# aosprey/mckpp-f90

Measured on AMD Instinct MI355X. Metric: column-steps/s at 1e5 cols x 60 levels, 1/2/4/8 GPU; % HBM roofline, higher is better.
Workload: dtype f64

## Files before the change

### mckpp_f90_amd/csrc/mckpp_device.h

```cpp
#pragma once
#include <hip/hip_runtime.h>
#include <stdint.h>

#define MCKPP_CS 24
#define MCKPP_CI 8
#define MCKPP_XS 8
enum { XS_RELAX_SST = 0, XS_SST0, XS_FCORR_TWOD, XS_RELAX_SAL, XS_RELAX_OCNT };

enum {
  CS_F = 0, CS_SSURF, CS_SREF, CS_SSREF, CS_OCDEPTH,
  CS_SFLUX1, CS_SFLUX2, CS_SFLUX3, CS_SFLUX4, CS_SFLUX5, CS_SFLUX6,
  CS_HMIXD0, CS_HMIXD1, CS_HMIX, CS_KMIX, CS_UREF, CS_VREF, CS_TREF,
  CS_RESET, CS_DAMPU, CS_DAMPV, CS_FREEZE, CS_FCORR, CS_SPARE1
};
enum { CI_OLD = 0, CI_NEW, CI_JERLOV, CI_INITFLAG, CI_STATUS, CI_NPASS, CI_LOCEAN, CI_IPT };

enum { MCKPP_MODE_STEP = 0, MCKPP_MODE_INIT = 1, MCKPP_MODE_PASS = 2, MCKPP_MODE_VMIX = 3 };

template <class T> using mckpp_ptr_plain = T *;
template <class T> using mckpp_ptr_global = __attribute__((address_space(1))) T *;

template <template <class> class P>
struct mckpp_kparams_t {
  int nz, nzp1, ncol, ld;
  int ntime, itermax, mode, diag;
  int L_SSref, LDD, clim_present;
  int l2pre;
  double hmixtolfrac, dto, grav, vonk, sice;
  double Vtc;
  double cg;
  double dm_nz;
  P<const double> zm, hm, tri0, tri1;
  P<const double> swfrac_tab;
  P<const double> swdk_tab;
  int ldc;
  int LRI;
  int solver_mode;
  int l3cap;
  P<const double> wtab;
  P<double> U, V, T, S;
  P<double> Us[2], Vs[2], Ts[2], Ss[2];
  P<const double> U_init, V_init;
  P<double> cs;
  P<int> ci;
  P<int> qhead;
  int nsteps_launch;
  int nqueues;
  int xcc_queue[16];
  P<const double> series;
  int series_rec0, ndtocn, l_rest;
  double flsn, el;
  P<int> qowner;
  P<int> done;
  P<unsigned long long> dbg;
  int ext, L_RELAX_SST, L_RELAX_CALCONLY, L_FCORR, L_FCORR_WITHZ, L_SFCORR, L_SFCORR_WITHZ;
  int L_RELAX_SAL, L_RELAX_OCNT, L_NO_FREEZE, L_NO_ISOTHERM, L_DAMP_CURR, iso_bot, dt_uvdamp, maxmodeadv;
  double iso_thresh;
  P<const double> dm;
  P<const double> hsum;
  P<const double> xs;
  P<const double> fcorr_withz, sfcorr_withz, ocnT_clim, sal_clim;
  P<double> tinc_fcorr, sinc_fcorr, ocnTcorr, scorr;
  P<const int> adv_i;
  P<const double> adv_d;
  P<double> rho, cp, buoy, talpha, sbeta, difm, difs, dift, ghat;
  P<double> wU1, wU2, wX1, wX2, wX3, wXNT1, Rig, dbloc, Shsq;
  P<double> scratch;
  size_t scratch_doubles;
  P<int> sync;
  int solo_after;
  int view_kmax;
  int solo_limit;
};
using mckpp_kparams = mckpp_kparams_t<mckpp_ptr_plain>;
using mckpp_kparams_dev = mckpp_kparams_t<mckpp_ptr_global>;
static_assert(sizeof(mckpp_kparams) == sizeof(mckpp_kparams_dev), "same layout");

struct mckpp_launch_info { int nblocks, threads, max_blocks_per_cu; size_t lds_bytes; };

hipError_t mckpp_launch_column_kernel_ps(const mckpp_kparams &p, const mckpp_kparams *dp, int num_cu,
                                         hipStream_t stream, mckpp_launch_info *info);
size_t mckpp_ps_scratch_doubles(int nzp1, int variant, int num_cu);
hipError_t mckpp_launch_xcc_probe(unsigned *mask, hipStream_t stream);
hipError_t mckpp_launch_eos_batch(int64_t n, const double *s, const double *t, const double *p,
                                  double *alpha, double *beta, double *sig0, double *cp,
                                  hipStream_t stream);
hipError_t mckpp_launch_div_batch(int64_t n, const double *num, const double *den, double *q, hipStream_t stream);
hipError_t mckpp_launch_exp_batch(int64_t n, const double *x, double *y, hipStream_t stream);
hipError_t mckpp_launch_bottomtemp(const mckpp_kparams &p, const double *bt, hipStream_t stream);
hipError_t mckpp_launch_fluxes(const mckpp_kparams &p, int ntime, const double *f8, int l_rest, double flsn,
                               double el, hipStream_t stream);
struct mckpp_pack_list { int nd, ni; int dslot[MCKPP_CS]; int islot[MCKPP_CI]; };
hipError_t mckpp_launch_unpack_sflux(const double *slabs, const int *ipt, double *cs, int64_t ncol, int64_t npts, hipStream_t stream);
hipError_t mckpp_launch_pack_records(const double *cs, const int *ci, const int *ipt, int64_t ncol, int64_t npts,
                                     const mckpp_pack_list &l, double *dout, int *iout, hipStream_t stream);
hipError_t mckpp_launch_out_sample(const double *src, int src_ld, int src_off, const double *cs, int add_sref,
                                   int64_t ncol, int nlev, int ld_out, double *sum, double *mn, double *mx, int first,
                                   double *inst, hipStream_t stream);
hipError_t mckpp_launch_window_mean(const double *sum, double *out, size_t n, double count, hipStream_t stream);
hipError_t mckpp_launch_gather_rows(const double *src3d, int64_t npts, int nlev, int lev_off,
                                    const int *ipt, int64_t ncol, double *dst, int ld, int dst_off,
                                    hipStream_t stream);
hipError_t mckpp_launch_scatter_rows(const double *src, int ld, int src_off, const int *ipt,
                                     int64_t ncol, double *dst3d, int64_t npts, int nlev, int lev_off,
                                     hipStream_t stream);
```

### mckpp_f90_amd/csrc/mckpp_kernels_ps.hip

```cpp
#include "mckpp_colmath.h"

#include <cstdio>
#include <cstdlib>
#include <type_traits>

namespace {

using namespace mckpp_dev;

enum { PS_EMPTY = 0, PS_ACTIVE = 1, PS_DONE = 2, PS_WAIT = 3  };
enum { F_NONE = 0, F_TRAP = 1, F_FINAL = 2 };

enum {
  C_B0 = 0, C_B0SOL, C_USTAR, C_UFRAC, C_UCUBE, C_HEK, C_WU01, C_WU02, C_WX01, C_WX02, C_WXNT0, C_UREFNZ, C_VREFNZ,
  C_RHO0CP0, C_RRC, X_T1 , X_S1, X_RHOH2O, X_RHOB,
  C_F, C_HMIXE, C_HMIXN, C_HBL, C_RHBL, C_STABLE, C_BFSFC, C_CASEA,
  C_GAT1, C_DAT1 = C_GAT1 + 3, C_DKM1 = C_DAT1 + 3,
  C_SREF = C_DKM1 + 3, C_SSURF, C_OCDEPTH, C_SFLUX1, C_SFLUX2, C_SFLUX3, C_SFLUX4, C_SFLUX5, C_SFLUX6,
  C_T1X ,
  C_JRFAC = C_T1X + 2, C_JA1, C_JA2, C_JRA1, C_JRA2 ,
  C_COUNT_USED,
  C_COUNT = C_COUNT_USED | 1
};
enum {
// ... 893 lines not shown
    c_t1[i] = p.tri1[i];
    c_rdz[i] = rcp_refine(p.zm[i] - p.zm[i + 1]);
    c_dtohk[i] = p.dto / p.hm[i];
  }
  if (tid == 0) { c_misc[0] = rcp_refine(p.hm[1]); c_misc[1] = rcp_refine(p.vonk); }
  for (int i = tid; i < W0 * I_COUNT; i += blockDim.x) sirec0[i] = 0;
  if (tid < 32) s_flags[tid] = tid == 3 ? nz : 0;
  const int mgr = 0;
  const int my_xcc = __builtin_amdgcn_s_getreg(((4 - 1) << 11) | 20 ) & 15;
  if (tid == 0 && p.nsteps_launch > 1) {
    int q = p.xcc_queue[my_xcc];
    if (q >= 0) {
      const int prev = atomicCAS((int *)p.qowner + q, 0, my_xcc + 1);
      if (prev != 0 && prev != my_xcc + 1) q = -1;
    }
    s_flags[7] = q;
  }

  const int nthreads = blockDim.x;
  const int nitems = W0 * L;
  const int nhelp = nthreads > 64 ? nthreads - 64 : 64, tid2 = nthreads > 64 ? tid - 64 : tid;
  const int nitems_lm = W0 * nzp1;
  const unsigned Wmagic = W0 > 1 ? 0xFFFFFFFFu / (unsigned)W0 + 1u : 0u;
  const int kmax_view = nthreads > 64 ? min(min((nthreads - 64) / L, (int)S_MAPMAX), p.view_kmax > 0 ? p.view_kmax : (int)S_MAPMAX) : 0;
  const bool solo_ok = kmax_view >= 1;
  const bool solo_perm = W0 == 1 && solo_ok;
  const bool solo_dyn = p.mode == MCKPP_MODE_STEP && solo_ok && !solo_perm && p.solo_limit > 0;
  bool sparse = false;
  int it0 = tid, it0_lm = tid, trip_base = nthreads;
  auto set_view = [&](int kv) {
    sparse = kv > 0;
    if (!sparse) { it0 = tid; it0_lm = tid; trip_base = nthreads; return; }
    trip_base = 0x20000000;
    const int i0 = tid - 64;
    it0 = 0x3fffffff; it0_lm = 0x3fffffff;
    if (i0 >= 0 && i0 < kv * L) {
      const int vs = (int)__umulhi((unsigned)i0, Lmagic);
      it0 = s_flags[S_MAP + vs] * L + (i0 - vs * L);
    }
    if (i0 >= 0 && i0 < kv * nzp1) {
      const int lk = i0 / kv;
      it0_lm = lk * W0 + s_flags[S_MAP + (i0 - lk * kv)];
    }
  };
  if (solo_perm && tid == 0) { s_flags[S_KVIEW] = 1; s_flags[S_MAP] = 0; }
  __syncthreads();
  if (solo_perm) set_view(1);

  const double lambda = 0.5;
  const double epsln16 = 1.e-16, Ricr = 0.30, eps01 = 0.1, cekman = 0.7, cmonob = 1.0, epsln20 = 1.e-20;
  const bool do_ocnint = p.mode == MCKPP_MODE_STEP || p.mode == MCKPP_MODE_PASS;
  const bool flux_diag = p.mode == MCKPP_MODE_STEP || p.mode == MCKPP_MODE_INIT;
  double rU = 0.0, rV = 0.0, rT = 0.0, rS = 0.0, r2U = 0.0, r2V = 0.0, r2T = 0.0, r2S = 0.0;
  const int LS = ps_scratch_ld(nzp1);
  const auto scr0 = p.scratch + (size_t)blockIdx.x * (size_t)W0 * (size_t)(4 * LS);

#define PS_ITEMS_PRAGMA _Pragma("clang loop unroll(disable)")
#define FOR_ITEMS                                                                         \
  PS_ITEMS_PRAGMA                                                                         \
  for (int it_ = it0, t_ = 0; it_ < nitems; it_ = tid2 >= 0 ? trip_base + t_ * nhelp + tid2 : nitems, ++t_) { \
    const int slot = (int)__umulhi((unsigned)it_, Lmagic);                                \
    const int k = it_ - slot * L + 1;                                                     \
    int *const si = sirec + slot * I_COUNT;                                               \
    if (!si[I_ACT]) continue;                                                             \
    double *const my = slots + slot * SS;                                                 \
    double *const sc = screc + slot * C_COUNT;                                            \
    const int col = si[I_COL];                                                            \
    const bool act = k <= nzp1, actz = k <= nz, virt1 = k == nzp1 + 1, virt2 = k == nzp1 + 2; \
    const bool is1 = k == 1, isnz = k == nz, isnzp1 = k == nzp1;                          \
    const int kr = act ? k : 1;                                                           \
    const size_t ro = (size_t)col * p.ld;                                                 \
    const auto xs_ = scr0 + (size_t)slot * (size_t)(4 * LS) + (kr - 1);    \
    const int first_ = t_;         \
    auto row = [&](int a) -> strided<ROWS> { return strided<ROWS>{my + a}; };             \
    (void)sc; (void)actz; (void)virt1; (void)virt2; (void)is1; (void)isnz; (void)isnzp1; (void)kr; (void)ro; (void)xs_; (void)first_; (void)row;
#define END_ITEMS }
#define FOR_ITEMS_BY_LEVEL                                                                \
  for (int j_ = it0_lm, t_ = 0; j_ < nitems_lm; j_ = tid2 >= 0 ? trip_base + t_ * nhelp + tid2 : nitems_lm, ++t_) { \
    const int it_ = t_ == 0 ? j_ : nitems_lm - 1 - (j_ - nthreads);                       \
    const int k = (W == 1 ? it_ : (int)__umulhi((unsigned)it_, Wmagic)) + 1;    \
    const int slot = it_ - (k - 1) * W;                                                   \
    int *const si = sirec + slot * I_COUNT;                                               \
    if (!si[I_ACT]) continue;                                                             \
    double *const my = slots + slot * SS;                                                 \
    double *const sc = screc + slot * C_COUNT;                                            \
    const int col = si[I_COL];                                                            \
    const bool act = true, actz = k <= nz;                                                \
    const bool is1 = k == 1, isnz = k == nz, isnzp1 = k == nzp1;                          \
    const size_t ro = (size_t)col * p.ld;                                                 \
    auto row = [&](int a) -> strided<ROWS> { return strided<ROWS>{my + a}; };             \
    (void)sc; (void)act; (void)actz; (void)is1; (void)isnz; (void)isnzp1; (void)ro; (void)row;

#define FOR_ITEMS_RISING                                                                  \
  for (int it_ = it0_lm, t_ = 0; it_ < nitems_lm; it_ = tid2 >= 0 ? trip_base + t_ * nhelp + tid2 : nitems_lm, ++t_) { \
    const int k = (W == 1 ? it_ : (int)__umulhi((unsigned)it_, Wmagic)) + 1;              \
    const int slot = it_ - (k - 1) * W;                                                   \
    int *const si = sirec + slot * I_COUNT;                                               \
    if (!si[I_ACT]) continue;                                                             \
    double *const my = slots + slot * SS;                                                 \
    double *const sc = screc + slot * C_COUNT;                                            \
    const bool actz = k <= nz, is1 = k == 1, isnz = k == nz;                              \
    auto row = [&](int a) -> strided<ROWS> { return strided<ROWS>{my + a}; };             \
    (void)sc; (void)actz; (void)is1; (void)isnz; (void)row;

  auto M0 = [&]() {
    int lane = lane_k; asm volatile("" : "+v"(lane));
// ... 323 lines not shown
              if (npass_try < p.itermax) { msc[C_HMIXE] = hmixn; go_on = true; }
              else if (hmixn > hmixe) { msc[C_HMIXE] = hmixn; go_on = true; }
            }
            if (!go_on) {
              if (npass_try > (p.itermax + 1)) status |= 2;
              fin = F_TRAP;
              msi[I_NVIOL] = 0;
            }
          }
          msi[I_MAYBE_NEXT] = (npass_try >= 3 && (iconv >= 2 || npass_try + 1 >= p.itermax)) ? 1 : 0;
        }
        msi[I_STATUS] = status; msi[I_NPASS_TRY] = npass_try; msi[I_ICONV] = iconv;
        msi[I_FIN] = fin;
        msi[I_L1A] = (l1_ahead && fin == F_NONE) ? 1 : 0;
        f_any = fin != F_NONE;
      }
    }
    const unsigned long long m = __ballot(f_any);
    if (lane == 0) s_flags[1] = m != 0ull ? 1 : 0;
#ifdef MCKPP_PS_STAMPS
    {
      const bool sg = lane < W && sirec[lane * I_COUNT + I_STATE] == PS_ACTIVE && sirec[lane * I_COUNT + I_ACT] && sirec[lane * I_COUNT + I_STRAG];
      const int n = __popcll(__ballot(sg));
      const int nact = __popcll(__ballot(lane < W && sirec[lane * I_COUNT + I_STATE] == PS_ACTIVE && sirec[lane * I_COUNT + I_ACT]));
      if (lane == 0 && n > 0) { atomicAdd((int *)p.sync + (sparse ? 1 : 2), n); atomicAdd((int *)p.sync + (sparse ? 3 : 4), 1); atomicAdd((int *)p.sync + (sparse ? 5 : 6), nact); }
    }
#endif
    if (solo_dyn && !sparse) {
      const int f_kv = s_flags[S_KVIEW], f_drain = s_flags[S_DRAIN];
      if (f_kv == 0 && f_drain) {
        const int *msi = sirec + (lane < W ? lane : 0) * I_COUNT;
        const bool on = lane < W && msi[I_STATE] == PS_ACTIVE && msi[I_ACT];
        const bool ok = on && msi[I_FIN] == F_NONE && (msi[I_STRAG] || msi[I_NPASS_TRY] > p.solo_after);
        const unsigned long long m_on = __ballot(on), m_ok = __ballot(ok);
        const int kn = __popcll(m_on);
        if (kn >= 1 && kn <= kmax_view && m_ok == m_on) {
          if (on) s_flags[S_MAP + __popcll(m_on & ((1ull << lane) - 1ull))] = lane;
          if (lane == 0) s_flags[S_GOVIEW] = kn;
        }
      }
    }
  };
  auto G_late = [&]() {
    int lane = lane_k; asm volatile("" : "+v"(lane));
    if (lane < W) {
      int *msi = sirec + lane * I_COUNT;
      if (msi[I_ACT]) {
        if (p.mode != MCKPP_MODE_INIT && msi[I_BAD]) msi[I_STATUS] = msi[I_STATUS] | 1;
        msi[I_BAD] = 0;
        msi[I_TINY] = 0;
        msi[I_MAYBE] = msi[I_MAYBE_NEXT];
      }
    }
  };

  auto ext_rhs = [&](double *my, const int *si, int col, int k, int kmixe, double To_k, double So_k, double &rhsT,
                     double &rhsS) {
    const double dto = p.dto;
    const auto xs = p.xs + (size_t)col * MCKPP_XS;
    const double rhok = my[k * ROWS + Q_RHO], cpk = my[k * ROWS + Q_CP];
    const size_t oin = (size_t)col * p.ld + (k - 1);
    if (k == 1) {
      if (p.L_RELAX_SST && !p.L_FCORR_WITHZ && !p.L_FCORR) {
        const double relax_sst = xs[XS_RELAX_SST], SST0 = xs[XS_SST0];
        double fc = 0.0;
        if (relax_sst > 1.e-10) {
          if (!p.L_RELAX_CALCONLY) rhsT = rhsT + dto * relax_sst * (SST0 - To_k) * p.dm[kmixe] / c_hm[1];
          fc = relax_sst * (SST0 - To_k) * p.dm[kmixe] * rhok * cpk;
        }
        p.cs[(size_t)col * MCKPP_CS + CS_FCORR] = fc;
      }
      if (p.L_FCORR && !p.L_RELAX_SST && !p.L_FCORR_WITHZ)
        rhsT = rhsT + dto * xs[XS_FCORR_TWOD] / (rhok * cpk * c_hm[1]);
    }
    double tinc = 0.;
    if (p.L_FCORR_WITHZ && !p.L_FCORR) tinc = dto * p.fcorr_withz[oin] / (rhok * cpk);
    if (p.L_RELAX_OCNT) tinc = tinc + dto * xs[XS_RELAX_OCNT] * (p.ocnT_clim[oin] - To_k);
    rhsT = rhsT + tinc;
    const double ocnTcorr = tinc * rhok * cpk / dto;
    const auto ai = p.adv_i + (size_t)col * (p.maxmodeadv + 1);
    const auto ad = p.adv_d + (size_t)col * (p.maxmodeadv + 1);
    const int nmode = ai[0];
    const int nzi = nz, km = kmixe;
    for (int im = 0; im < nmode; ++im) {
      const int mode = ai[1 + im];
      if (mode <= 0) continue;
      const double fact = dto * ad[im] * 0.033;
      if (mode == 1) {
        if (k == 1) rhsS = rhsS + fact / c_hm[1];
      } else if (mode == 2) {
        const double delta = p.hsum[km - 1];
        if (k <= km - 1) rhsS = rhsS + fact / delta;
      } else if (mode == 3) {
        const double delta = p.hsum[nzi];
        if (k <= nzi) rhsS = rhsS + fact / delta;
      } else if (mode == 4) {
        const int nzend = nzi - 1;
        int n1 = 0;
        do { n1 = n1 + 1; } while (c_zm[n1] >= -100. && n1 < nzp1);
        double delta = 0.0;
        for (int n = n1; n <= nzend; ++n) delta = delta + c_hm[n];
        if (k >= n1 && k <= nzend) rhsS = rhsS + fact / delta;
      } else if (mode == 5) {
        if (k == nzi) rhsS = rhsS + fact / c_hm[nzi];
      } else if (mode == 6 || mode == 7) {
        int n1, n2 = 0;
// ... 616 lines not shown
          if (wv == wv2) ps_thomas2_uts_fwd<XV, -1>(W, slots, SS, nz, sirec + I_ACT, I_COUNT, sirec + I_BAD, I_COUNT, lane);
        }
      } else {
        if (wv == mgr) ps_thomas2_uts_fwd<XV, 1>(W, slots, SS, nz, sirec + I_ACT, I_COUNT, sirec + I_BAD, I_COUNT, lane);
        if (wv == wv2) ps_thomas2_uts_fwd<XV, -1>(W, slots, SS, nz, sirec + I_ACT, I_COUNT, sirec + I_BAD, I_COUNT, lane);
      }
      STAMP(24);
      __syncthreads();
      if (wv == mgr) ps_thomas2_uts_back<XV, 1>(W, slots, SS, nz, sirec + I_ACT, I_COUNT, sirec + I_BAD, I_COUNT, lane);
      if (wv == wv2) ps_thomas2_uts_back<XV, -1>(W, slots, SS, nz, sirec + I_ACT, I_COUNT, sirec + I_BAD, I_COUNT, lane);
    }
    STAMP(16);
    __syncthreads();
    STAMP(17);

    if (do_ocnint) {
      FOR_ITEMS
        if (!act) continue;
        const size_t o = ro + (k - 1);
        const double Uo = p.U[o], Vo = p.V[o];
        const double dto = p.dto, f = sc[C_F];
        const strided<ROWS> yU = row(Q_YU), yV = row(Q_YV);
        if (actz) {
          const double pk = row(Q_DM)[k], qk = row(Q_GM)[k], gk = row(ps_sysrows<XV>::gam_m)[k];
          double betk;
          if constexpr (SM == 0) {
            betk = (k == 1) ? 1. + pk : ((1. + pk) + qk) + qk * gk;
          } else {
            const int m = nz >> 1;
            const double gk1 = row(ps_sysrows<XV>::gam_m)[k + 1];
            if (k <= m) {
              betk = (k == 1) ? 1. + pk : ((1. + pk) + qk) + qk * gk;
              row(Q_DM)[k] = gk1;
            } else {
              betk = (k == nz) ? (1. + pk) + qk : ((1. + pk) + qk) + pk * gk1;
              row(Q_GM)[k] = pk;
              row(Q_DM)[k] = gk;
            }
          }
          if (betk == 0.) betk = 1.E-12;
          row(Q_BET)[k] = betk;
          row(Q_DT)[k] = rcp_refine(betk);
          const double un = yU[k];
          double rhsV;
          if (k == 1) rhsV = Vo - dto * (f * .5 * (Uo + un) + div_fast(sc[C_WU02], c_hm[1], c_misc[0]));
          else rhsV = Vo - dto * f * .5 * (Uo + un);
          if (k == nz) rhsV = rhsV + c_t1[nz] * 0.0001  * p.V[ro + (nzp1 - 1)];
          yV[k] = rhsV;
        } else {
          yV[k] = Vo;
        }
      END_ITEMS
    }
    STAMP(18);
    __syncthreads();
    STAMP(19);

    const bool late_on_mgr = SM != 0 || nthreads <= 64;
    if (wv == mgr) {
      if (do_ocnint) {
        if constexpr (SM == 0) {
          ps_thomas_v_fwd(W, slots, SS, ROWS, nz, sirec + I_ACT, I_COUNT, lane);
          STAMP(25);
          ps_thomas_v_back(W, slots, SS, ROWS, ps_sysrows<XV>::gam_m, nz, sirec + I_ACT, I_COUNT, lane);
        } else {
          ps_thomas2_v(W, slots, SS, ROWS, ps_sysrows<XV>::gam_m, nz, sirec + I_ACT, I_COUNT, sirec + I_BAD, I_COUNT, lane);
        }
      }
      if (late_on_mgr) G_late();
    } else {
      if (!late_on_mgr && wv == (nthreads >> 6) - 1) G_late();
      if (l1_ahead) {
      FOR_ITEMS
        if (!si[I_L1A]) continue;
        L1_item(k, kr, si, my, sc, ro, act, virt1, virt2, is1, xs_, first_, L1_ALL_BUT_V);
      END_ITEMS
      }
    }
    STAMP(20);
    __syncthreads();
    STAMP(21);
    finishing = s_flags[1];
    if (finishing) {

    FOR_ITEMS
      if (!act) continue;
      if (si[I_FIN] != F_TRAP) continue;
      const size_t o = ro + (k - 1);
      const double U = row(Q_YU)[k], V = row(Q_YV)[k], T = row(Q_YT)[k], S = row(Q_YS)[k], tk1 = row(Q_YT)[k + 1];
      const double Uo = p.U[o], Vo = p.V[o], To = p.T[o], So = p.S[o];
      const bool v = actz && (__builtin_fabs(U) >= 10 || __builtin_fabs(V) >= 10 || __builtin_fabs(T - tk1) >= 10);
      if (v) atomicAdd(&si[I_NVIOL], 1);
      const double hk = c_hm[k];
      row(Q_DM)[k] = (U - Uo) * (U - Uo) * hk / p.dm_nz;
      row(Q_DT)[k] = (V - Vo) * (V - Vo) * hk / p.dm_nz;
      row(Q_DS)[k] = (T - To) * (T - To) * hk / p.dm_nz;
      row(Q_GM)[k] = (S - So) * (S - So) * hk / p.dm_nz;
    END_ITEMS
    __syncthreads();
    STAMP(26);
    if (wv == mgr) {
      if (lane < W) sirec[lane * I_COUNT + I_NOVER] = 0;
      for (int l = lane; l < 4 * W; l += 64) {
        const int ms = l >> 2, mq = l & 3;
        int *msi = sirec + ms * I_COUNT;
        if (msi[I_ACT] && msi[I_FIN] == F_TRAP && msi[I_NVIOL] == 0) {
          const strided<ROWS> t{slots + ms * SS + (mq == 3 ? (int)Q_GM : (int)Q_DM + mq)};
          double sum = 0.;
          int q = 1;
          for (; q + 7 <= nzp1; q += 8) {
            const double a0 = t[q], a1 = t[q + 1], a2 = t[q + 2], a3 = t[q + 3], a4 = t[q + 4], a5 = t[q + 5], a6 = t[q + 6], a7 = t[q + 7];
            sum = sum + a0; sum = sum + a1; sum = sum + a2; sum = sum + a3; sum = sum + a4; sum = sum + a5; sum = sum + a6; sum = sum + a7;
          }
          for (; q <= nzp1; ++q) sum = sum + t[q];
          sum = __builtin_sqrt(sum);
          if (sum >= 1.0) atomicAdd(&msi[I_NOVER], 1);
        }
      }
      if (lane < W) {
        int *msi = sirec + lane * I_COUNT;
        double *msc = screc + lane * C_COUNT;
        if (msi[I_ACT] && msi[I_FIN] == F_TRAP) {
          int comp_flag = 0, status = msi[I_STATUS], nreset = msi[I_NRESET];
          double f = msc[C_F];
          const int nviol = msi[I_NVIOL];
          if (nviol > 0) {
            comp_flag = 1;
            for (int i = 0; i < nviol; ++i) f = f * 1.01;
          } else {
            const int nover = msi[I_NOVER];
            if (nover > 0) {
              comp_flag = 1;
              for (int i = 0; i < nover; ++i) f = f * 1.01;
            }
          }
          if (comp_flag) { status |= 4; msc[C_F] = f; }
          nreset = nreset + 1;
          if (nreset > 10) status |= 8;
          msi[I_COMP] = comp_flag; msi[I_STATUS] = status; msi[I_NRESET] = nreset;
          if (comp_flag && nreset <= 10) {
            msi[I_FIN] = F_NONE; msi[I_LOAD] = 2; msi[I_NPASS_TRY] = 0; msi[I_ICONV] = 0; msi[I_MAYBE] = 0;
          } else {
            msi[I_FIN] = F_FINAL;
            msi[I_NU] = 0; msi[I_NV] = 0; msi[I_NF] = 0;
          }
        }
      }
    }
    __syncthreads();
    STAMP(27);
    FOR_ITEMS
      if (!act) continue;
      if (si[I_FIN] != F_FINAL) continue;
      const bool fstep = p.mode == MCKPP_MODE_STEP;
      const bool sol = do_ocnint;
      const size_t o = ro + (k - 1);
      double U = 0, V = 0, T = 0, S = 0, uk1 = 0, vk1 = 0, tk1 = 0, sk1 = 0;
      if (act) {
        if (sol) { U = row(Q_YU)[k]; V = row(Q_YV)[k]; T = row(Q_YT)[k]; S = row(Q_YS)[k]; }
        else { U = p.U[o]; V = p.V[o]; T = p.T[o]; S = p.S[o]; }
      }
      if (actz && p.diag && flux_diag) {
        if (sol) { uk1 = row(Q_YU)[k + 1]; vk1 = row(Q_YV)[k + 1]; tk1 = row(Q_YT)[k + 1]; sk1 = row(Q_YS)[k + 1]; }
        else { uk1 = p.U[o + 1]; vk1 = p.V[o + 1]; tk1 = p.T[o + 1]; sk1 = p.S[o + 1]; }
      }
      if (p.diag) {
        const double wX0_1 = sc[C_WX01], wX0_2 = sc[C_WX02];
        const double rho0cp0 = sc[C_RHO0CP0], sflux3 = sc[C_SFLUX3];
        const size_t od = ro + k;
        {
          if (actz) {
            const double dfm = p.difm[od], dfs = p.difs[od], dft = p.dift[od], gh = p.ghat[od];
            const double talpha = flux_diag ? p.talpha[od] : 0.0, sbeta = flux_diag ? p.sbeta[od] : 0.0;
            const double swdk = (ntime >= 1) ? p.swdk_tab[si[I_JER] * p.ldc + k] : 0.0;
            p.wXNT1[od] = (ntime >= 1) ? -sflux3 * swdk / rho0cp0 : 0.0;
            if (flux_diag) {
              double deltaz = 0.5 * (c_hm[k] + c_hm[k + 1]);
              double wX1 = -dfs * ((T - tk1) / deltaz - gh * wX0_1);
              double wX2 = -dfs * ((S - sk1) / deltaz - gh * wX0_2);
              if (p.LDD) wX1 = -dft * ((T - tk1) / deltaz - gh * wX0_1);
              p.wX1[od] = wX1; p.wX2[od] = wX2;
              p.wX3[od] = p.grav * (talpha * wX1 - sbeta * wX2);
              p.wU1[od] = -dfm * (U - uk1) / deltaz;
              p.wU2[od] = -dfm * (V - vk1) / deltaz;
            }
          }
        }
        if (is1) {
          p.difm[ro] = 0.0; p.difs[ro] = 0.0; p.dift[ro] = 0.0;
          p.wU1[ro] = sc[C_WU01]; p.wU2[ro] = sc[C_WU02];
          p.wX1[ro] = wX0_1; p.wX2[ro] = wX0_2; p.wX3[ro] = -sc[C_B0];
          p.wXNT1[ro] = sc[C_WXNT0];
        }
      }
      if (fstep && is1) {
        const auto cs = p.cs + (size_t)col * MCKPP_CS;
        cs[CS_UREF] = U; cs[CS_VREF] = V; cs[CS_TREF] = T;
        cs[CS_SSURF] = p.L_SSref ? cs[CS_SSREF] : S + sc[C_SREF];
      }
      if constexpr (EXT) {
        if (fstep && p.L_DAMP_CURR && act) {
          const double rr = (double)p.dt_uvdamp * (86400. / p.dto);
          double a = 0.99 * __builtin_fabs(U), b = (U * U) / rr;
          if (b < a) atomicAdd(&si[I_NU], 1);
          row(Q_YU)[k] = U - dsign(dmin2(a, b), U);
          a = 0.99 * __builtin_fabs(V); b = (V * V) / rr;
          if (b < a) atomicAdd(&si[I_NV], 1);
          row(Q_YV)[k] = V - dsign(dmin2(a, b), V);
        }
      }
    END_ITEMS
    __syncthreads();
    STAMP(28);
    FOR_ITEMS
      if (!act) continue;
      if (!(si[I_FIN] == F_FINAL && p.mode == MCKPP_MODE_STEP)) continue;
      const size_t o = ro + (k - 1);
      const int newi = 1 - si[I_NEW];
      double U = 0, V = 0, T = 0, S = 0;
      if (act) { U = row(Q_YU)[k]; V = row(Q_YV)[k]; T = row(Q_YT)[k]; S = row(Q_YS)[k]; }
      if (act) { p.Us[newi][o] = U; p.Vs[newi][o] = V; p.Ts[newi][o] = T; p.Ss[newi][o] = S; }
      if (si[I_COMP] && act) {
        if (p.clim_present) { T = p.ocnT_clim[o]; S = p.sal_clim[o]; row(Q_YT)[k] = T; row(Q_YS)[k] = S; }
        U = p.U_init[o]; V = p.V_init[o];
        row(Q_YU)[k] = U; row(Q_YV)[k] = V;
      }
      if constexpr (EXT) {
        if (si[I_LOCEAN] && p.L_NO_FREEZE && act) {
          double xt = p.tinc_fcorr[ro + k];
          if (T < -1.8) { xt = xt + (-1.8 - T); T = -1.8; row(Q_YT)[k] = T; atomicAdd(&si[I_NF], 1); }
          p.tinc_fcorr[ro + k] = xt;
        }
      }
    END_ITEMS
    if constexpr (EXT) {
      __syncthreads();
      FOR_ITEMS
        if (!act) continue;
        if (!(si[I_FIN] == F_FINAL && p.mode == MCKPP_MODE_STEP && si[I_LOCEAN] && p.L_NO_ISOTHERM)) continue;
        if (k >= 2 && act) {
          const double dz = c_zm[k] - c_zm[k - 1];
          row(Q_DM)[k] = __builtin_fabs((row(Q_YT)[k] - row(Q_YT)[k - 1])) * dz;
          row(Q_DT)[k] = dz;
        }
      END_ITEMS
      __syncthreads();
    }
    FOR_ITEMS
      if (!act) continue;
      if (si[I_FIN] != F_FINAL) continue;
      const auto cs = p.cs + (size_t)col * MCKPP_CS;
      const auto ci = p.ci + (size_t)col * MCKPP_CI;
      const size_t o = ro + (k - 1);
      if (p.mode == MCKPP_MODE_STEP) {
        double reset_out = (double)si[I_NRESET];
        if (si[I_COMP]) reset_out = 999.;
        bool iso_reset = false;
        if constexpr (EXT) {
          if (si[I_LOCEAN] && p.L_NO_ISOTHERM) {
            const strided<ROWS> tD = row(Q_DM), tZ = row(Q_DT);
            double dtdz_total = 0., dz_total = 0.;
            for (int q = 2; q <= p.iso_bot; ++q) {
              dtdz_total = dtdz_total + tD[q];
              dz_total = dz_total + tZ[q];
            }
// ... 203 lines not shown
```

### mckpp_f90_amd/csrc/mckpp_runtime.cpp

```cpp
#include "../../include/mckpp_hip.h"
#include "mckpp_device.h"
#include "mckpp_math.h"

#include <cmath>
#include <cstdarg>
#include <cstdio>
#include <cstdlib>
#include <cstring>
#include <string>
#include <thread>
#include <vector>

namespace {

thread_local std::string g_err;

int fail(const char *fmt, ...)
{
  char buf[512];
  va_list ap;
  va_start(ap, fmt);
  vsnprintf(buf, sizeof buf, fmt, ap);
  va_end(ap);
  g_err = buf;
// ... 28 lines not shown

enum { P_U = 0, P_V, P_T, P_S, P_US0, P_US1, P_VS0, P_VS1, P_TS0, P_TS1, P_SS0, P_SS1, P_UINIT, P_VINIT, P_COUNT };
enum { E_FCORR_WITHZ = 0, E_SFCORR_WITHZ, E_OCNT_CLIM, E_SAL_CLIM, E_COUNT };
enum { O_TINC = 0, O_SINC, O_OCNTCORR, O_SCORR, O_COUNT };
enum { D_RHO = 0, D_CP, D_BUOY, D_TALPHA, D_SBETA, D_DIFM, D_DIFS, D_DIFT, D_GHAT, D_WU1, D_WU2,
       D_WX1, D_WX2, D_WX3, D_WXNT1, D_RIG, D_DBLOC, D_SHSQ, D_COUNT };

const double jer_rfac[6] = {0, 0.58, 0.62, 0.67, 0.77, 0.78};
const double jer_a1[6] = {0, 0.35, 0.6, 1.0, 1.5, 1.4};
const double jer_a2[6] = {0, 23.0, 20.0, 17.0, 14.0, 7.9};

}

enum { QBLOCK_INTS = 64 };

struct mckpp_hip_ctx {
  int device = 0;
  hipStream_t stream = nullptr;
  hipEvent_t ev0 = nullptr, ev1 = nullptr;
  bool timed = false;
  int nlaunch = 0;
  int nkernels = 0;
  mckpp_const_c c{};
  int nz = 0, nzp1 = 0, lpl = 1, ld = 64, ldc = 72;
  double Vtc = 0, cg = 0, dm_nz = 0;
  std::vector<double> h_swfrac_tab, h_swdk_tab;
  double *d_zm = nullptr, *d_hm = nullptr, *d_tri0 = nullptr, *d_tri1 = nullptr;
  double *d_swfrac_tab = nullptr, *d_swdk_tab = nullptr;
  double2 *d_wtab = nullptr;
  int64_t npts = 0, ncol = 0;
  std::vector<int> ipt;
  int *d_ipt = nullptr;
  double *d_prof[P_COUNT] = {};
  double *d_diag[D_COUNT] = {};
  bool ext = false;
  bool ext_kernel = false;
  double *d_ext_in[E_COUNT] = {};
  double *d_ext_out[O_COUNT] = {};
  double *d_xs = nullptr, *d_adv_d = nullptr, *d_dm = nullptr, *d_hsum = nullptr;
  int *d_adv_i = nullptr;
  std::vector<int> wsel{0, 1, 2, 3, 4};
  std::vector<double *> d_wacc;
  int window_count = 0;
  double *d_cs = nullptr;
  int *d_ci = nullptr;
  int *d_qhead = nullptr;
  int view_kmax = 0;
  int solo_after = 12, solo_limit = 8;
  int *d_done = nullptr;
  bool multistep = true;
  int nqueues = 0;
  int xcc_queue[16];
  int l3cap = 0;
  int solver_mode = 0;
  unsigned long long *d_dbg = nullptr;
  mckpp_kparams *d_params = nullptr;
  mckpp_kparams *h_params = nullptr;
  hipEvent_t ev_params[2] = {nullptr, nullptr};
  unsigned params_seq = 0;
  double *d_scratch = nullptr;
  size_t scratch_doubles = 0;
  int num_cu = 256;
  int l2pre = 0;
  double *d_series = nullptr;
  int series_rec0 = 0, series_nrec = 0;
  mckpp_launch_info last_launch{};
  double *d_stage = nullptr;
  size_t stage_elems = 0;
  hipStream_t copy_stream = nullptr;
  double *d_xfer[2] = {nullptr, nullptr};
  size_t xfer_elems[2] = {0, 0};
  hipEvent_t ev_lay[2] = {nullptr, nullptr}, ev_copy[2] = {nullptr, nullptr};
  unsigned xfer_seq = 0;
  std::vector<std::pair<const void *, size_t>> pinned;
  std::vector<std::pair<const void *, size_t>> unpinnable;
  double *h_cs = nullptr, *h_f = nullptr;
  int *h_ci = nullptr;
  size_t h_f_elems = 0;
  hipEvent_t ev_f = nullptr;
  double *d_pack = nullptr, *h_pack = nullptr;
  int diag = 1;
  bool ext_inputs_resident = false;
};

extern "C" {

const char *mckpp_hip_last_error(void) { return g_err.c_str(); }

#ifndef MCKPP_BUILD_ID
#define MCKPP_BUILD_ID "unknown"
#endif
const char *mckpp_hip_build_id(void) { return MCKPP_BUILD_ID; }
#ifndef MCKPP_BUILD_COMPILER
#define MCKPP_BUILD_COMPILER "unknown"
#endif
const char *mckpp_hip_build_compiler(void) { return MCKPP_BUILD_COMPILER; }

int mckpp_hip_device_count(void)
{
  int n = 0;
  hipError_t e = hipGetDeviceCount(&n);
  if (e != hipSuccess) return fail("hipGetDeviceCount: %s", hipGetErrorString(e));
  return n;
}

void mckpp_host_lookup(double vonk, double *wmt, double *wst)
// ... 88 lines not shown
  HIPCHK(hipMalloc(&h->d_qhead, QBLOCK_INTS * sizeof(int)));
  h->solo_after = 12;
  h->solo_limit = std::max(2, h->num_cu / 32);
  if (const char *e = getenv("MCKPP_SOLO")) { if (atoi(e) == 0) h->solo_limit = 0; }
  if (const char *e = getenv("MCKPP_SOLO_LIMIT")) h->solo_limit = std::max(0, atoi(e));
  if (const char *e = getenv("MCKPP_SOLO_AFTER")) h->solo_after = std::max(0, atoi(e));
  if (const char *e = getenv("MCKPP_VIEW_KMAX")) h->view_kmax = std::max(0, atoi(e));
  {
    HIPCHK(hipMemsetAsync(h->d_qhead, 0, sizeof(int), h->stream));
    HIPCHK(mckpp_launch_xcc_probe(reinterpret_cast<unsigned *>(h->d_qhead), h->stream));
    unsigned mask = 0;
    HIPCHK(hipMemcpyAsync(&mask, h->d_qhead, sizeof mask, hipMemcpyDeviceToHost, h->stream));
    HIPCHK(hipStreamSynchronize(h->stream));
    h->nqueues = 0;
    for (int i = 0; i < 16; ++i) h->xcc_queue[i] = (mask >> i & 1u) ? h->nqueues++ : -1;
    if (h->nqueues == 0) h->multistep = false;
    if (const char *e = getenv("MCKPP_XCC_DROP")) {
      const unsigned drop = (unsigned)strtoul(e, nullptr, 0);
      for (int i = 0; i < 16; ++i) if (drop >> i & 1u) h->xcc_queue[i] = -1;
    }
    if (getenv("MCKPP_PS_VERBOSE"))
      fprintf(stderr, "[mckpp] XCC ids seen by the probe: mask 0x%x, %d queues\n", mask, h->nqueues);
  }
  HIPCHK(hipMalloc(&h->d_params, sizeof(mckpp_kparams)));
  h->scratch_doubles = mckpp_ps_scratch_doubles(nzp1, h->ext_kernel ? (c->LDD ? 2 : 1) : 0, h->num_cu);
  HIPCHK(hipMalloc(&h->d_scratch, h->scratch_doubles * sizeof(double)));
  HIPCHK(hipMemset(h->d_scratch, 0, h->scratch_doubles * sizeof(double)));
  if (getenv("MCKPP_STAMP")) {
    HIPCHK(hipMalloc(&h->d_dbg, 32 * sizeof(unsigned long long)));
    HIPCHK(hipMemset(h->d_dbg, 0, 32 * sizeof(unsigned long long)));
  }
  HIPCHK(hipEventCreate(&h->ev0));
  HIPCHK(hipEventCreate(&h->ev1));
  HIPCHK(hipStreamCreateWithFlags(&h->copy_stream, hipStreamNonBlocking));
  for (int b = 0; b < 2; ++b) {
    HIPCHK(hipEventCreateWithFlags(&h->ev_lay[b], hipEventDisableTiming));
    HIPCHK(hipEventCreateWithFlags(&h->ev_copy[b], hipEventDisableTiming));
    HIPCHK(hipEventCreateWithFlags(&h->ev_params[b], hipEventDisableTiming));
  }
  HIPCHK(hipEventCreateWithFlags(&h->ev_f, hipEventDisableTiming));
  HIPCHK(hipHostMalloc(&h->h_params, 2 * sizeof(mckpp_kparams), hipHostMallocDefault));

  const int ldc = h->ldc, nz = h->nz, n1 = c->nztmax + 1;
  std::vector<double> zm(ldc, 0.0), hm(ldc, 0.0), t0(ldc, 0.0), t1(ldc, 0.0);
  for (int k = 1; k <= nzp1; ++k) { zm[k] = c->zm[k - 1]; hm[k] = c->hm[k - 1]; }
  for (int k = 0; k <= nz; ++k) { t0[k] = c->tri[k]; t1[k] = c->tri[n1 + k]; }
  h->dm_nz = c->dm[nz];
  {
    int nref = 0;
    for (int k = 1; k <= nz; ++k) nref += c->zm[k - 1] > 0.1 * c->zm[nz - 1];
    h->l2pre = (nref >= 16 && !c->LDD) ? 1 : 0;
    if (const char *e = getenv("MCKPP_L2PRE")) h->l2pre = (atoi(e) != 0 && !c->LDD) ? 1 : 0;
    if (const char *e = getenv("MCKPP_L3_CAP")) h->l3cap = atoi(e) > 0 ? atoi(e) : 0;
    h->solver_mode = solver_mode_env;
    if (const char *e = getenv("MCKPP_MULTISTEP")) h->multistep = atoi(e) != 0 && h->nqueues > 0;
  }
  {
    std::vector<double> dm(ldc, 0.0), hs(ldc, 0.0);
    for (int k = 0; k <= nz; ++k) dm[k] = c->dm[k];
    double acc = 0.0;
    for (int n = 1; n <= nzp1; ++n) { acc = acc + hm[n]; hs[n] = acc; }
    HIPCHK(hipMalloc(&h->d_dm, ldc * sizeof(double)));
    HIPCHK(hipMemcpy(h->d_dm, dm.data(), ldc * sizeof(double), hipMemcpyHostToDevice));
    HIPCHK(hipMalloc(&h->d_hsum, ldc * sizeof(double)));
    HIPCHK(hipMemcpy(h->d_hsum, hs.data(), ldc * sizeof(double), hipMemcpyHostToDevice));
  }
  h->h_swfrac_tab.assign((size_t)6 * ldc, 0.0);
  h->h_swdk_tab.assign((size_t)6 * ldc, 0.0);
  for (int jw = 1; jw <= 5; ++jw) {
    for (int l = 1; l <= nzp1; ++l) {
      const double rmin = -80.;
      double r1 = zm[l] * 1.0 / jer_a1[jw]; r1 = r1 > rmin ? r1 : rmin;
      double r2 = zm[l] * 1.0 / jer_a2[jw]; r2 = r2 > rmin ? r2 : rmin;
      h->h_swfrac_tab[(size_t)jw * ldc + l] = jer_rfac[jw] * mckpp_exp(r1) + (1. - jer_rfac[jw]) * mckpp_exp(r2);
    }
    for (int k = 0; k <= nz; ++k) {
      const double z = -c->dm[k];
      h->h_swdk_tab[(size_t)jw * ldc + k] =
          jer_rfac[jw] * mckpp_exp(z / jer_a1[jw]) + (1.0 - jer_rfac[jw]) * mckpp_exp(z / jer_a2[jw]);
    }
  }
  {
    const double cv = 1.6, cs = 98.96, epsilon = 0.1, Ricr = 0.30, cstar = 5.0;
    h->Vtc = cv * std::sqrt(0.2 / cs / epsilon) / (c->vonk * c->vonk) / Ricr;
    h->cg = cstar * c->vonk * std::pow(cs * c->vonk * epsilon, 1. / 3.);
  }
  const size_t nt = (size_t)(MCKPP_NI + 2) * (MCKPP_NJ + 2);
  std::vector<double2> wtab(nt);
  for (size_t i = 0; i < nt; ++i) wtab[i] = make_double2(c->wmt[i], c->wst[i]);

  auto up = [&](double **dst, const double *src, size_t n) -> hipError_t {
    hipError_t e = hipMalloc(dst, n * sizeof(double));
    if (e != hipSuccess) return e;
    return hipMemcpy(*dst, src, n * sizeof(double), hipMemcpyHostToDevice);
  };
  HIPCHK(up(&h->d_zm, zm.data(), ldc));
  HIPCHK(up(&h->d_hm, hm.data(), ldc));
  HIPCHK(up(&h->d_tri0, t0.data(), ldc));
  HIPCHK(up(&h->d_tri1, t1.data(), ldc));
  HIPCHK(up(&h->d_swfrac_tab, h->h_swfrac_tab.data(), (size_t)6 * ldc));
  HIPCHK(up(&h->d_swdk_tab, h->h_swdk_tab.data(), (size_t)6 * ldc));
  HIPCHK(hipMalloc(&h->d_wtab, nt * sizeof(double2)));
  HIPCHK(hipMemcpy(h->d_wtab, wtab.data(), nt * sizeof(double2), hipMemcpyHostToDevice));
  h->c.zm = h->c.hm = h->c.dm = h->c.tri = h->c.wmt = h->c.wst = nullptr;
  g.p = nullptr;
  *out = h;
// ... 385 lines not shown
  if (ensure_stage(h, bt.size())) return -1;
  HIPCHK(hipMemcpyAsync(h->d_stage, bt.data(), bt.size() * sizeof(double), hipMemcpyHostToDevice, h->stream));
  mckpp_kparams p;
  fill_params(h, p, 0, MCKPP_MODE_STEP);
  HIPCHK(mckpp_launch_bottomtemp(p, h->d_stage, h->stream));
  HIPCHK(hipStreamSynchronize(h->stream));
  return 0;
}

int mckpp_hip_release_host_arrays(mckpp_hip_handle h)
{
  if (!h) return fail("null handle");
  HIPCHK(hipSetDevice(h->device));
  if (xfer_finish(h)) return -1;
  unpin_all(h);
  return 0;
}

int mckpp_hip_set_diagnostics(mckpp_hip_handle h, int on)
{
  if (!h) return fail("null handle");
  h->diag = on ? 1 : 0;
  return 0;
}

int mckpp_hip_set_solver_mode(mckpp_hip_handle h, int mode)
{
  if (!h) return fail("null handle");
  if (mode < 0 || mode > 1) return fail("mckpp_hip_set_solver_mode: unknown solver mode (0: the reference's order, 1: two-ended)");
  h->solver_mode = mode;
  return 0;
}

int mckpp_hip_get_solver_mode(mckpp_hip_handle h) { return h ? h->solver_mode : fail("null handle"); }

static void fill_params(mckpp_hip_ctx *h, mckpp_kparams &p, int ntime, int mode)
{
  memset(&p, 0, sizeof p);
  p.nz = h->nz; p.nzp1 = h->nzp1; p.ncol = (int)h->ncol; p.ld = h->ld;
  p.ntime = ntime; p.itermax = h->c.itermax; p.mode = mode; p.diag = h->diag;
  p.L_SSref = h->c.L_SSref; p.LDD = h->c.LDD; p.clim_present = h->c.clim_present;
  p.l2pre = h->l2pre; p.LRI = h->c.LRI ? 1 : 0; p.l3cap = h->l3cap; p.solver_mode = h->solver_mode;
  p.hmixtolfrac = h->c.hmixtolfrac; p.dto = h->c.dto; p.grav = h->c.grav; p.vonk = h->c.vonk; p.sice = h->c.sice;
  p.Vtc = h->Vtc; p.cg = h->cg; p.dm_nz = h->dm_nz;
  p.zm = h->d_zm; p.hm = h->d_hm; p.tri0 = h->d_tri0; p.tri1 = h->d_tri1;
  p.swfrac_tab = h->d_swfrac_tab; p.swdk_tab = h->d_swdk_tab; p.ldc = h->ldc; p.wtab = reinterpret_cast<const double *>(h->d_wtab);
  p.U = h->d_prof[P_U]; p.V = h->d_prof[P_V]; p.T = h->d_prof[P_T]; p.S = h->d_prof[P_S];
  p.Us[0] = h->d_prof[P_US0]; p.Us[1] = h->d_prof[P_US1]; p.Vs[0] = h->d_prof[P_VS0]; p.Vs[1] = h->d_prof[P_VS1];
  p.Ts[0] = h->d_prof[P_TS0]; p.Ts[1] = h->d_prof[P_TS1]; p.Ss[0] = h->d_prof[P_SS0]; p.Ss[1] = h->d_prof[P_SS1];
  p.U_init = h->d_prof[P_UINIT]; p.V_init = h->d_prof[P_VINIT];
  p.cs = h->d_cs; p.ci = h->d_ci; p.qhead = h->d_qhead; p.dbg = h->d_dbg;
  p.nsteps_launch = 1; p.done = h->d_done; p.nqueues = h->nqueues; p.qowner = h->d_qhead + 16;
  p.sync = h->d_qhead + 32; p.solo_after = h->solo_after; p.solo_limit = h->solo_limit; p.view_kmax = h->view_kmax;
  for (int i = 0; i < 16; ++i) p.xcc_queue[i] = h->xcc_queue[i];
  p.ext = h->ext_kernel ? 1 : 0;
  p.L_RELAX_SST = h->c.L_RELAX_SST; p.L_RELAX_CALCONLY = h->c.L_RELAX_CALCONLY; p.L_FCORR = h->c.L_FCORR;
  p.L_FCORR_WITHZ = h->c.L_FCORR_WITHZ; p.L_SFCORR = h->c.L_SFCORR; p.L_SFCORR_WITHZ = h->c.L_SFCORR_WITHZ;
  p.L_RELAX_SAL = h->c.L_RELAX_SAL; p.L_RELAX_OCNT = h->c.L_RELAX_OCNT; p.L_NO_FREEZE = h->c.L_NO_FREEZE;
  p.L_NO_ISOTHERM = h->c.L_NO_ISOTHERM; p.L_DAMP_CURR = h->c.L_DAMP_CURR; p.iso_bot = h->c.iso_bot;
  p.dt_uvdamp = h->c.dt_uvdamp; p.maxmodeadv = h->c.maxmodeadv; p.iso_thresh = h->c.iso_thresh;
  p.dm = h->d_dm; p.hsum = h->d_hsum; p.xs = h->d_xs; p.adv_i = h->d_adv_i; p.adv_d = h->d_adv_d;
  p.fcorr_withz = h->d_ext_in[E_FCORR_WITHZ]; p.sfcorr_withz = h->d_ext_in[E_SFCORR_WITHZ];
  p.ocnT_clim = h->d_ext_in[E_OCNT_CLIM]; p.sal_clim = h->d_ext_in[E_SAL_CLIM];
  p.tinc_fcorr = h->d_ext_out[O_TINC]; p.sinc_fcorr = h->d_ext_out[O_SINC];
  p.ocnTcorr = h->d_ext_out[O_OCNTCORR]; p.scorr = h->d_ext_out[O_SCORR];
  p.rho = h->d_diag[D_RHO]; p.cp = h->d_diag[D_CP]; p.buoy = h->d_diag[D_BUOY];
  p.talpha = h->d_diag[D_TALPHA]; p.sbeta = h->d_diag[D_SBETA];
  p.difm = h->d_diag[D_DIFM]; p.difs = h->d_diag[D_DIFS]; p.dift = h->d_diag[D_DIFT]; p.ghat = h->d_diag[D_GHAT];
  p.wU1 = h->d_diag[D_WU1]; p.wU2 = h->d_diag[D_WU2];
  p.wX1 = h->d_diag[D_WX1]; p.wX2 = h->d_diag[D_WX2]; p.wX3 = h->d_diag[D_WX3]; p.wXNT1 = h->d_diag[D_WXNT1];
  p.Rig = h->d_diag[D_RIG]; p.dbloc = h->d_diag[D_DBLOC]; p.Shsq = h->d_diag[D_SHSQ];
  p.scratch = h->d_scratch; p.scratch_doubles = h->scratch_doubles;
}

struct forced_run { int ndtocn, l_rest; double flsn, el; };

static int run(mckpp_hip_ctx *h, int ntime, int nsteps, int mode, const forced_run *forced = nullptr)
{
  if (!h) return fail("null handle");
  if (h->ncol == 0) { h->nlaunch = 0; h->timed = false; return 0; }
  if (h->ext && !h->ext_inputs_resident)
    return fail("optional-physics context: the relaxation / correction / advection inputs are not resident "
                "(after mckpp_hip_load_restart call mckpp_hip_update_ancillaries before stepping)");
  HIPCHK(hipSetDevice(h->device));
  {
    const unsigned slot = h->params_seq++ & 1u;
    HIPCHK(hipEventSynchronize(h->ev_params[slot]));
    fill_params(h, h->h_params[slot], ntime, mode);
    HIPCHK(hipMemcpyAsync(h->d_params, &h->h_params[slot], sizeof(mckpp_kparams), hipMemcpyHostToDevice, h->stream));
    HIPCHK(hipEventRecord(h->ev_params[slot], h->stream));
  }
  HIPCHK(hipEventRecord(h->ev0, h->stream));
  if (mode == MCKPP_MODE_STEP && nsteps > 1 && ntime >= 1 && h->multistep) {
    if (!h->d_done) HIPCHK(hipMalloc(&h->d_done, 2 * (size_t)h->ncol * sizeof(int)));
    const int per_launch = (int)std::max<int64_t>(1, ((int64_t)1 << 30) / h->ncol);
    for (int i = 0; i < nsteps; i += per_launch) {
      const int n = nsteps - i < per_launch ? nsteps - i : per_launch;
      const unsigned slot = h->params_seq++ & 1u;
      HIPCHK(hipEventSynchronize(h->ev_params[slot]));
      fill_params(h, h->h_params[slot], ntime + i, mode);
      h->h_params[slot].nsteps_launch = n;
      if (forced) {
        mckpp_kparams &q = h->h_params[slot];
        q.series = h->d_series; q.series_rec0 = h->series_rec0; q.ndtocn = forced->ndtocn; q.l_rest = forced->l_rest;
        q.flsn = forced->flsn; q.el = forced->el;
      }
// ... 1017 lines not shown
```

Before: 34.17 million.

## Move trapezoid finish work under the M5 phase and drop a barrier

```diff
diff --git a/mckpp_f90_amd/csrc/mckpp_device.h b/mckpp_f90_amd/csrc/mckpp_device.h
--- a/mckpp_f90_amd/csrc/mckpp_device.h
+++ b/mckpp_f90_amd/csrc/mckpp_device.h
@@ -71,6 +71,7 @@
   int solo_after;
   int view_kmax;
   int solo_limit;
+  int fin_m5;
 };
 using mckpp_kparams = mckpp_kparams_t<mckpp_ptr_plain>;
 using mckpp_kparams_dev = mckpp_kparams_t<mckpp_ptr_global>;
diff --git a/mckpp_f90_amd/csrc/mckpp_kernels_ps.hip b/mckpp_f90_amd/csrc/mckpp_kernels_ps.hip
--- a/mckpp_f90_amd/csrc/mckpp_kernels_ps.hip
+++ b/mckpp_f90_amd/csrc/mckpp_kernels_ps.hip
@@ -969,6 +969,7 @@
   const bool do_ocnint = p.mode == MCKPP_MODE_STEP || p.mode == MCKPP_MODE_PASS;
   const bool flux_diag = p.mode == MCKPP_MODE_STEP || p.mode == MCKPP_MODE_INIT;
   double rU = 0.0, rV = 0.0, rT = 0.0, rS = 0.0, r2U = 0.0, r2V = 0.0, r2T = 0.0, r2S = 0.0;
+  double rX = 0.0, r2X = 0.0;
   const int LS = ps_scratch_ld(nzp1);
   const auto scr0 = p.scratch + (size_t)blockIdx.x * (size_t)W0 * (size_t)(4 * LS);
 
@@ -1398,6 +1399,52 @@
         msi[I_MAYBE] = msi[I_MAYBE_NEXT];
       }
     }
+  };
+
+  const bool fin_m5 = p.fin_m5 != 0 && p.mode == MCKPP_MODE_STEP;
+  auto fin_early = [&](const int k, double *const my, double *const sc, const int *const si, const size_t ro, const int col,
+                       const bool actz, const bool is1, const int first_) {
+    auto row = [&](int a) -> strided<ROWS> { return strided<ROWS>{my + a}; };
+    const size_t o = ro + (k - 1);
+    const double U = row(Q_YU)[k], T = row(Q_YT)[k], S = row(Q_YS)[k];
+    const double Uo = p.U[o], Vo = p.V[o], To = p.T[o], So = p.S[o];
+    const double hk = c_hm[k];
+    const double tU = (U - Uo) * (U - Uo) * hk / p.dm_nz, tT = (T - To) * (T - To) * hk / p.dm_nz,
+                 tS = (S - So) * (S - So) * hk / p.dm_nz;
+    double dfm = 0.0;
+    if (p.diag) {
+      const double wX0_1 = sc[C_WX01], wX0_2 = sc[C_WX02];
+      const double rho0cp0 = sc[C_RHO0CP0], sflux3 = sc[C_SFLUX3];
+      const size_t od = ro + k;
+      if (actz) {
+        const double tk1 = row(Q_YT)[k + 1], sk1 = row(Q_YS)[k + 1], uk1 = row(Q_YU)[k + 1];
+        dfm = p.difm[od];
+        const double dfs = p.difs[od], dft = p.dift[od], gh = p.ghat[od];
+        const double talpha = p.talpha[od], sbeta = p.sbeta[od];
+        const double swdk = (ntime >= 1) ? p.swdk_tab[si[I_JER] * p.ldc + k] : 0.0;
+        p.wXNT1[od] = (ntime >= 1) ? -sflux3 * swdk / rho0cp0 : 0.0;
+        double deltaz = 0.5 * (c_hm[k] + c_hm[k + 1]);
+        double wX1 = -dfs * ((T - tk1) / deltaz - gh * wX0_1);
+        double wX2 = -dfs * ((S - sk1) / deltaz - gh * wX0_2);
+        if (p.LDD) wX1 = -dft * ((T - tk1) / deltaz - gh * wX0_1);
+        p.wX1[od] = wX1; p.wX2[od] = wX2;
+        p.wX3[od] = p.grav * (talpha * wX1 - sbeta * wX2);
+        p.wU1[od] = -dfm * (U - uk1) / deltaz;
+      }
+      if (is1) {
+        p.difm[ro] = 0.0; p.difs[ro] = 0.0; p.dift[ro] = 0.0;
+        p.wU1[ro] = sc[C_WU01]; p.wU2[ro] = sc[C_WU02];
+        p.wX1[ro] = wX0_1; p.wX2[ro] = wX0_2; p.wX3[ro] = -sc[C_B0];
+        p.wXNT1[ro] = sc[C_WXNT0];
+      }
+    }
+    if (is1) {
+      const auto cs = p.cs + (size_t)col * MCKPP_CS;
+      cs[CS_UREF] = U; cs[CS_TREF] = T;
+      cs[CS_SSURF] = p.L_SSref ? cs[CS_SSREF] : S + sc[C_SREF];
+    }
+    if (first_ == 0) { rU = tU; rV = Vo; rT = tT; rS = tS; rX = dfm; }
+    else { r2U = tU; r2V = Vo; r2T = tT; r2S = tS; r2X = dfm; }
   };
 
   auto ext_rhs = [&](double *my, const int *si, int col, int k, int kmixe, double To_k, double So_k, double &rhsT,
@@ -2120,6 +2167,12 @@
         }
       END_ITEMS
     }
+    if (fin_m5 && wv == mgr && s_flags[1]) {
+      FOR_ITEMS
+        if (!act || first_ >= 2 || si[I_FIN] != F_TRAP) continue;
+        fin_early(k, my, sc, si, ro, col, actz, is1, first_);
+      END_ITEMS
+    }
     STAMP(18);
     __syncthreads();
     STAMP(19);
@@ -2138,10 +2191,11 @@
       if (late_on_mgr) G_late();
     } else {
       if (!late_on_mgr && wv == (nthreads >> 6) - 1) G_late();
-      if (l1_ahead) {
+      const bool fin_here = fin_m5 && s_flags[1];
+      if (l1_ahead || fin_here) {
       FOR_ITEMS
-        if (!si[I_L1A]) continue;
-        L1_item(k, kr, si, my, sc, ro, act, virt1, virt2, is1, xs_, first_, L1_ALL_BUT_V);
+        if (si[I_L1A]) L1_item(k, kr, si, my, sc, ro, act, virt1, virt2, is1, xs_, first_, L1_ALL_BUT_V);
+        else if (fin_here && act && first_ < 2 && si[I_FIN] == F_TRAP) fin_early(k, my, sc, si, ro, col, actz, is1, first_);
       END_ITEMS
       }
     }
@@ -2156,10 +2210,24 @@
       if (si[I_FIN] != F_TRAP) continue;
       const size_t o = ro + (k - 1);
       const double U = row(Q_YU)[k], V = row(Q_YV)[k], T = row(Q_YT)[k], S = row(Q_YS)[k], tk1 = row(Q_YT)[k + 1];
-      const double Uo = p.U[o], Vo = p.V[o], To = p.T[o], So = p.S[o];
       const bool v = actz && (__builtin_fabs(U) >= 10 || __builtin_fabs(V) >= 10 || __builtin_fabs(T - tk1) >= 10);
       if (v) atomicAdd(&si[I_NVIOL], 1);
       const double hk = c_hm[k];
+      if (fin_m5 && first_ < 2) {
+        const double Vo = first_ == 0 ? rV : r2V, dfm = first_ == 0 ? rX : r2X;
+        row(Q_DM)[k] = first_ == 0 ? rU : r2U;
+        row(Q_DT)[k] = (V - Vo) * (V - Vo) * hk / p.dm_nz;
+        row(Q_DS)[k] = first_ == 0 ? rT : r2T;
+        row(Q_GM)[k] = first_ == 0 ? rS : r2S;
+        if (actz && p.diag) {
+          const double vk1 = row(Q_YV)[k + 1];
+          double deltaz = 0.5 * (c_hm[k] + c_hm[k + 1]);
+          p.wU2[ro + k] = -dfm * (V - vk1) / deltaz;
+        }
+        if (is1) p.cs[(size_t)col * MCKPP_CS + CS_VREF] = V;
+        continue;
+      }
+      const double Uo = p.U[o], Vo = p.V[o], To = p.T[o], So = p.S[o];
       row(Q_DM)[k] = (U - Uo) * (U - Uo) * hk / p.dm_nz;
       row(Q_DT)[k] = (V - Vo) * (V - Vo) * hk / p.dm_nz;
       row(Q_DS)[k] = (T - To) * (T - To) * hk / p.dm_nz;
@@ -2228,6 +2296,8 @@
         if (sol) { U = row(Q_YU)[k]; V = row(Q_YV)[k]; T = row(Q_YT)[k]; S = row(Q_YS)[k]; }
         else { U = p.U[o]; V = p.V[o]; T = p.T[o]; S = p.S[o]; }
       }
+      const bool early = fin_m5 && first_ < 2;
+      if (!early) {
       if (actz && p.diag && flux_diag) {
         if (sol) { uk1 = row(Q_YU)[k + 1]; vk1 = row(Q_YV)[k + 1]; tk1 = row(Q_YT)[k + 1]; sk1 = row(Q_YS)[k + 1]; }
         else { uk1 = p.U[o + 1]; vk1 = p.V[o + 1]; tk1 = p.T[o + 1]; sk1 = p.S[o + 1]; }
@@ -2266,6 +2336,7 @@
         cs[CS_UREF] = U; cs[CS_VREF] = V; cs[CS_TREF] = T;
         cs[CS_SSURF] = p.L_SSref ? cs[CS_SSREF] : S + sc[C_SREF];
       }
+      }
       if constexpr (EXT) {
         if (fstep && p.L_DAMP_CURR && act) {
           const double rr = (double)p.dt_uvdamp * (86400. / p.dto);
@@ -2278,7 +2349,7 @@
         }
       }
     END_ITEMS
-    __syncthreads();
+    if (!fin_m5 || EXT || nitems > trip_base + nhelp) __syncthreads();
     STAMP(28);
     FOR_ITEMS
       if (!act) continue;
diff --git a/mckpp_f90_amd/csrc/mckpp_runtime.cpp b/mckpp_f90_amd/csrc/mckpp_runtime.cpp
--- a/mckpp_f90_amd/csrc/mckpp_runtime.cpp
+++ b/mckpp_f90_amd/csrc/mckpp_runtime.cpp
@@ -104,6 +104,7 @@
   int nqueues = 0;
   int xcc_queue[16];
   int l3cap = 0;
+  int fin_m5 = 1;
   int solver_mode = 0;
   unsigned long long *d_dbg = nullptr;
   mckpp_kparams *d_params = nullptr;
@@ -298,6 +299,7 @@
     h->l2pre = (nref >= 16 && !c->LDD) ? 1 : 0;
     if (const char *e = getenv("MCKPP_L2PRE")) h->l2pre = (atoi(e) != 0 && !c->LDD) ? 1 : 0;
     if (const char *e = getenv("MCKPP_L3_CAP")) h->l3cap = atoi(e) > 0 ? atoi(e) : 0;
+    if (const char *e = getenv("MCKPP_FINISH_UNDER_M5")) h->fin_m5 = atoi(e) != 0 ? 1 : 0;
     h->solver_mode = solver_mode_env;
     if (const char *e = getenv("MCKPP_MULTISTEP")) h->multistep = atoi(e) != 0 && h->nqueues > 0;
   }
@@ -789,6 +791,7 @@
   p.cs = h->d_cs; p.ci = h->d_ci; p.qhead = h->d_qhead; p.dbg = h->d_dbg;
   p.nsteps_launch = 1; p.done = h->d_done; p.nqueues = h->nqueues; p.qowner = h->d_qhead + 16;
   p.sync = h->d_qhead + 32; p.solo_after = h->solo_after; p.solo_limit = h->solo_limit; p.view_kmax = h->view_kmax;
+  p.fin_m5 = h->fin_m5;
   for (int i = 0; i < 16; ++i) p.xcc_queue[i] = h->xcc_queue[i];
   p.ext = h->ext_kernel ? 1 : 0;
   p.L_RELAX_SST = h->c.L_RELAX_SST; p.L_RELAX_CALCONLY = h->c.L_RELAX_CALCONLY; p.L_FCORR = h->c.L_FCORR;
```

After: 34.24 million, median of 6. About the same (+0.2%).
